# videosegmentation/video_segment

Hardware: AMD Instinct MI355X
Metric: over-segmented frames/sec at 1080p (higher is better)
Workload: dtype f32

## Files before the change

video_segment_amd/csrc/dense_graph.cpp:

```cpp
#include "dense_graph.h"
#include "scan_device.h"

#include <algorithm>
#include <chrono>
#include <cmath>
#include <cstring>
#include <atomic>
#include <functional>
#include <thread>
#include <unordered_set>

namespace vsg {

namespace {
template <class T>
DevBuf<T>& Grow(DevBuf<T>& b, size_t n) {
  if (b.size() < n) b.alloc(n + n / 2 + 1024);
  return b;
}
double NowMs() {
  using clk = std::chrono::steady_clock;
  return std::chrono::duration<double, std::milli>(clk::now().time_since_epoch()).count();
}
template <class T>
// ... 399 lines not shown
    S.seg_key = act_.seg_key;
    S.seg_cnt = act_.seg_cnt;
    S.seg_off = act_.seg_off;
    S.lead_pos = act_.lead_pos;
    S.l_ra = act_.l_ra;
    S.l_rb = act_.l_rb;
    S.l_gpos = act_.l_gpos;
    S.bk_ds = act_.bk_ds;
    S.bk_cons = act_.bk_cons;
    S.bk_flags = act_.bk_flags;
    S.cub_temp = cub_temp_.get();
    S.cub_temp_bytes = cub_temp_.size();
    S.scan = ScanScratch{scan_sums_.get(), stream_};
    S.active_cap = (int)std::min<size_t>(scratch_active_, 0x7fffffff);
  };
  bind_scratch();
  S.grow_active = [this, bind_scratch, &diag_slab_growths, &diag_slab_ms](long long need) {
    const double tg0 = NowMs();
    VSG_HIP(hipStreamSynchronize(stream_));
    VSG_HIP(hipStreamSynchronize(aux_stream_));
    VSG_HIP(hipStreamSynchronize(aux2_stream_));
    const size_t before = scratch_active_;
    EnsureActiveScratch((size_t)need);
    bind_scratch();
    ++diag_slab_growths;
    diag_slab_ms += NowMs() - tg0;
    if (getenv("VSG_DEBUG_STATS")) {
      std::fprintf(stderr, "[vsg] stage scratch: %zu -> %zu active edges (needed %lld), %.2f ms\n", before,
                   scratch_active_, need, NowMs() - tg0);
    }
    return true;
  };
  S.num_active = scalars_.get();
  S.num_segs = scalars_.get() + 1;
  S.node_key_bits = 1;
  while (S.node_key_bits < 32 && ((size_t)1 << S.node_key_bits) < N) ++S.node_key_bits;
  {
    const size_t words = 4 * ((scratch_edges_ + 255) / 256) + 4;
    S.masks.active = filter_masks_.get();
    S.masks.settled = filter_masks_.get() + words;
    S.masks.tentative = filter_masks_.get() + 2 * words;
    S.masks.block_cnt = block_cnt_.get();
    S.block_off = block_off_.get();
  }
  S.force_rollback = getenv("VSG_FORCE_ROLLBACK") ? 1 : 0;
  S.small_seg = getenv("VSG_SMALL_SEG") ? std::max(1, atoi(getenv("VSG_SMALL_SEG"))) : 24;
  S.wide_min = getenv("VSG_WIDE_MIN") ? atoi(getenv("VSG_WIDE_MIN")) : 0;
  S.wide_waves = getenv("VSG_WIDE_WAVES") ? atoi(getenv("VSG_WIDE_WAVES")) : 4;
  S.chain_relax = getenv("VSG_CHAIN_RELAX") ? atoi(getenv("VSG_CHAIN_RELAX")) : 1;
  const int hubs_default = getenv("VSG_HUBS") ? atoi(getenv("VSG_HUBS")) : 1;
  S.hubs = hubs_default;
  S.hub_excl = hub_excl_.get();
  S.hub_max_splits = getenv("VSG_HUB_SPLITS") ? std::max(0, atoi(getenv("VSG_HUB_SPLITS"))) : kHubMaxSplits;
  S.hub_cut_min_work = getenv("VSG_CUT_MIN_WORK") ? atoi(getenv("VSG_CUT_MIN_WORK")) : 0;
  S.hub_cut_ratio = getenv("VSG_CUT_RATIO") ? std::max(0, atoi(getenv("VSG_CUT_RATIO"))) : 1500;
  S.hub_check = (getenv("VSG_HUB_CHECK") && atoi(getenv("VSG_HUB_CHECK")) != 0) ? 1 : 0;
  VSG_HIP(hipMemsetAsync(hub8_.get(), 0, N, stream_));
  S.spine_min = getenv("VSG_SPINE_MIN") ? atoi(getenv("VSG_SPINE_MIN")) : 2048;
  {
    const double want = 1.15 * (double)wh_ * (double)capacity_frames_;
    const int by_graph = (int)std::min<double>(std::max<double>(want, 1 << 20), 120 << 20);
    S.spine_max_edges = getenv("VSG_SPINE_MAX_EDGES") ? atoi(getenv("VSG_SPINE_MAX_EDGES"))
                                                      : std::max(by_graph, spine_max_edges_grown_);
  }
  S.spine_off = 0;
  if (spine_limit_bucket_ != 0x7fffffff && ++spine_limit_age_ > 8) {
    spine_limit_bucket_ = 0x7fffffff;
    spine_limit_age_ = 0;
  }
  S.spine_limit_bucket = &spine_limit_bucket_;
  int spine_low_failed[2] = {0, 0}, spine_low_skip[2] = {0, 0};
  for (int b = 0; b < 2; ++b) {
    if (spine_low_cooldown_[b] > 0) {
      --spine_low_cooldown_[b];
      spine_low_skip[b] = 1;
    }
  }
  S.spine_low_failed = spine_low_failed;
  S.spine_low_skip = spine_low_skip;
  S.spine_nested_factor = getenv("VSG_SPINE_NESTED") ? std::max(1, atoi(getenv("VSG_SPINE_NESTED"))) : 1;
  S.spine_debug = getenv("VSG_SPINE_DEBUG") ? 1 : 0;
  S.spine_check = getenv("VSG_SPINE_CHECK") ? 1 : 0;
  S.rank_split_min = getenv("VSG_RANK_SPLIT_MIN") ? atoi(getenv("VSG_RANK_SPLIT_MIN")) : (1 << 20);
  S.spine_fast = getenv("VSG_SPINE_FAST") ? atoi(getenv("VSG_SPINE_FAST")) : 2;
  S.spine_fast_min = getenv("VSG_SPINE_FAST_MIN") ? atoi(getenv("VSG_SPINE_FAST_MIN")) : 32768;
  if (S.spine_min > 0) {
    const size_t ints = SpinePoolInts((size_t)S.spine_max_edges);
    if (spine_pool_.size() < ints) spine_pool_.alloc(ints);
  }
  S.spine_pool = spine_pool_.get();
  S.spine_pool_ints = spine_pool_.size();
  S.grow_spine_pool = [this, &S, &diag_spine_growths, &diag_spine_ms](long long edges) {
    if (getenv("VSG_SPINE_MAX_EDGES") || edges >= (120ll << 20)) return false;
    const long long want = std::min<long long>(edges + edges / 8, 120ll << 20);
    const long long nodes = (long long)wh_ * (long long)std::max(capacity_frames_, 1);
    const size_t ints = SpinePoolInts((size_t)want) + (size_t)(29 * std::min(want, nodes));
    if (ints <= spine_pool_.size()) return false;
    const double tg0 = NowMs();
    size_t free_b = 0, total_b = 0;
    VSG_HIP(hipMemGetInfo(&free_b, &total_b));
    if (free_b + spine_pool_.size() * sizeof(int32_t) < 2 * ints * sizeof(int32_t)) {
      int dev = 0;
      VSG_HIP(hipGetDevice(&dev));
      CacheTrim(dev);
      VSG_HIP(hipMemGetInfo(&free_b, &total_b));
      if (free_b + spine_pool_.size() * sizeof(int32_t) < 2 * ints * sizeof(int32_t)) return false;
    }
    VSG_HIP(hipStreamSynchronize(stream_));
    VSG_HIP(hipStreamSynchronize(aux_stream_));
    VSG_HIP(hipStreamSynchronize(aux2_stream_));
    spine_pool_.alloc(ints);
    ++diag_spine_growths;
    diag_spine_ms += NowMs() - tg0;
    S.spine_pool = spine_pool_.get();
    S.spine_pool_ints = spine_pool_.size();
    S.spine_max_edges = (int)want;
    spine_max_edges_grown_ = S.spine_max_edges;
    return true;
  };
  S.nmap[0] = label_uf_.get();
  S.nmap[1] = label_img_.get();
  S.nmap[2] = adjust_.get();
  S.aux_stream = aux_stream_;
  S.aux2_stream = aux2_stream_;
  S.aux_fork = aux_fork_;
  S.aux_join = aux_join_;
  S.use_rle = getenv("VSG_RLE") ? atoi(getenv("VSG_RLE")) : 1;
  S.wave_dbg = getenv("VSG_WAVE_DBG") ? atoi(getenv("VSG_WAVE_DBG")) : 0;
  S.wave_debug = (S.wave_dbg != 0 || getenv("VSG_DEBUG_STAGES") || getenv("VSG_DEBUG_STATS")) ? 1 : 0;
  optimistic_stages_ = 0;
  rollbacks_ = 0;
  S.optimistic_stages = &optimistic_stages_;
  S.rollbacks = &rollbacks_;
  S.cc = cc_.get();
  S.stats = stats_.get();
  ev_used_ = 0;
  ev_wave_.clear();
  ev_filter_.clear();
  ev_spine_.clear();
  S.ev_pool = &ev_pool_;
  S.ev_wave = &ev_wave_;
  S.ev_filter = &ev_filter_;
  S.ev_spine = &ev_spine_;
  S.ev_used = &ev_used_;
  S.mail = &mail_;
  S.zeros = &zero_pool_;
  S.main_stream = stream_;

  MergeParams P;
  P.spatial_survivors = pass == 2 ? kept_spatial_pass_.get() : nullptr;
  P.W = W_;
  P.H = H_;
  P.num_lists = L;
  P.min_region_size = min_region_size;
  P.force_merge_weight = l1_ ? 0.002f : 0.001f;
  const float scale = 2048.0f / (1.0f + 1e-6f);
  P.inv_scale = (float)(1.0 / (double)scale);
  auto largest_s = [](double t, bool inclusive) {
    auto ok = [&](float s) {
      const double r = (double)std::sqrt(s);
      return inclusive ? r <= t : r < t;
    };
    float s = (float)(t * t);
    while (!ok(s)) s = std::nextafter(s, 0.0f);
    while (ok(std::nextafter(s, 10.0f))) s = std::nextafter(s, 10.0f);
    return s;
// ... 1182 lines not shown
```

video_segment_amd/csrc/device_graph.h:

```cpp
#ifndef VSG_DEVICE_GRAPH_H_
#define VSG_DEVICE_GRAPH_H_

#include <functional>

#include "common.h"

namespace vsg {

constexpr uint8_t kFlagFinalized = 1;
constexpr uint8_t kFlagNoDesc = 2;
constexpr uint8_t kFlagTentative = 4;
constexpr uint8_t kFlagHub = 8;
constexpr uint8_t kFlagHubBroken = 16;
constexpr uint8_t kFlagHubExcluded = 32;
constexpr int kHubExclCap = 16384;
constexpr int kHubMaxAttempts = 4;
constexpr int kHubMaxSplits = 64;
constexpr int kHubCutCap = 64;
constexpr int kHubListInts = 4 + kHubExclCap + 3 * kHubCutCap;

struct NodeArrays {
  int32_t* parent;
  float4* desc_sz;
  int32_t* cons;
  uint8_t* flags;
  uint8_t* hub8;
};

struct ListDesc {
  const uint32_t* slots;
  uint8_t* kept;
  const int32_t* prev_idx;
  const int32_t* offsets;
  int32_t type;
  int32_t base_a;
  int32_t base_b;
  int32_t n;
};

struct MergeParams {
  int W, H;
  int num_lists;
  int min_region_size;
  float force_merge_weight;
  float inv_scale;
  float s_lt_005, s_lt_02, s_le_015;
  const uint8_t* spatial_survivors;
};

void UploadSpaceWeights(const float* w49, hipStream_t stream);
void LaunchMinMax(const uint8_t* bgr, size_t stride, int W, int H, int* mm, hipStream_t s);
void LaunchBilateral(const uint8_t* bgr, size_t stride, int W, int H, const float* lut,
                     float scale, float* planes, hipStream_t s);
void LaunchGaussian3(const uint8_t* bgr, size_t stride, int W, int H, float k0, float k1, float* planes,
                     hipStream_t s);
void LaunchConvertPlanar(const uint8_t* bgr, size_t stride, int W, int H, float* planes,
                         hipStream_t s);
void LaunchInterleavedToPlanar(const float* in, size_t n, float* planes, hipStream_t s);
void LaunchPlanarToInterleaved(const float* planes, size_t n, float* out, hipStream_t s);
size_t EdgeSortHistInts(size_t n_px);
size_t EdgeSortSumInts(size_t n_px);
void LaunchSpatialKeys(const float* feat, int W, int H, int l1, uint16_t* keys, int32_t* hist,
                       hipStream_t s);
void LaunchTemporalKeys(const float* cur, const float* prev, const float* flow, int W, int H,
                        int l1, int is_virtual, uint16_t* keys, int32_t* prev_idx, int32_t* hist,
                        hipStream_t s);
void LaunchBucketSort(const uint16_t* keys, size_t n_px, int per_px, int32_t* hist, int32_t* sums,
                      int32_t* offsets, uint32_t* slots_out, hipStream_t s);
void LaunchInitNodes(const float* feat, size_t n, int base, const int32_t* cons_in,
                     NodeArrays nodes, hipStream_t s);
void LaunchInitVirtualNodes(const int32_t* labels, size_t n, int base, int num_labels,
                            int32_t* first_scratch, NodeArrays nodes, hipStream_t s);

constexpr int kScanMaxTiles = 4096;
struct ScanScratch {
  int32_t* sums;
  hipStream_t owner = nullptr;
};

size_t SortPairsU32HandTempBytes(int n);
void SortPairsU32Hand(void* temp, size_t temp_bytes, const uint32_t* keys_in, uint32_t* keys_out,
                      const uint32_t* vals_in, uint32_t* vals_out, int n, int end_bit, hipStream_t s);
size_t SortPairsU32LibTempBytes(int n);
void SortPairsU32Lib(void* temp, size_t temp_bytes, const uint32_t* keys_in, uint32_t* keys_out,
                     const uint32_t* vals_in, uint32_t* vals_out, int n, int end_bit, hipStream_t s);
size_t SortPairsU32TempBytes(int n);
void SortPairsU32(void* temp, size_t temp_bytes, const uint32_t* keys_in, uint32_t* keys_out,
                  const uint32_t* vals_in, uint32_t* vals_out, int n, int end_bit, hipStream_t s);
size_t SortKeysU64TempBytes(int n);
void SortKeysU64(void* temp, size_t temp_bytes, const unsigned long long* in,
                 unsigned long long* out, int n,
                 hipStream_t s);
size_t UniqueU64TempBytes(int n);
void UniqueU64(void* temp, size_t temp_bytes, const unsigned long long* in,
               unsigned long long* out,
               int32_t* num_out, int n, hipStream_t s);

constexpr int kMailValues = 4;
struct MailSlot {
  unsigned long long* dev;
  volatile unsigned long long* host;
  unsigned seq;
// ... 13 lines not shown
  m.next = (m.next + 1) % m.slots;
  return s;
}
void MailWait(const MailSlot& slot, int count, int* values, hipStream_t s);
void MailRegisterGraph(int delta);
int MailYieldMode();
struct MailWaitCounters {
  long long waits = 0;
  double wait_ms = 0, longest_ms = 0;
};
MailWaitCounters MailWaitSnapshot();
void MailWaitResetLongest();
void LaunchMailPost(const MailSlot& slot, const int32_t* p0, const int32_t* p1, const int32_t* p2,
                    const int32_t* p3, hipStream_t s);

constexpr size_t kZeroArenaInts = 1024;
struct ZeroPool {
  int32_t* base = nullptr;
  size_t cap = 0, used = 0;
  bool second_half = false;
  size_t arena_used = 0;
};

struct FilterMasks {
  unsigned long long* active;
  unsigned long long* settled;
  unsigned long long* tentative;
  int32_t* block_cnt;
};
struct FilterSegs {
  const int32_t* start;
  const int32_t* list;
  const int32_t* pos0;
  int n;
};
struct MergeScratch {
  int active_cap;
  std::function<bool(long long need)> grow_active;
  int32_t* e_ra;
  int32_t* e_rb;
  uint32_t* e_gpos;
  int32_t* e_active;
  int32_t* e_apos;
  FilterMasks masks;
  int32_t* block_off;
  int32_t* a_ra;
  int32_t* a_rb;
  uint32_t* a_gpos;
  uint32_t* a_comp;
  uint32_t* a_idx;
  uint32_t* s_comp;
  uint32_t* s_idx;
  uint32_t* seg_key;
  int32_t* seg_cnt;
  int32_t* seg_off;
  int32_t* num_active;
  int32_t* num_segs;
  float4* bk_ds;
  int32_t* bk_cons;
  uint8_t* bk_flags;
  int force_rollback;
  int32_t* lead_pos;
  int32_t* l_ra;
  int32_t* l_rb;
  uint32_t* l_gpos;
  int use_rle;
  int group_hi;
  const int32_t* bucket_prefix;
  const int32_t* bucket_prefix_host;
  const int32_t* bucket_base_host;
  const int32_t* list_off_host;
  int32_t* seg_dev;
  size_t seg_cap;
  std::vector<int32_t>* seg_host;
  int spine_min;
  int spine_off;
  int* spine_low_failed;
  const int* spine_low_skip;
  int* spine_limit_bucket;
  int spine_nested_factor;
  int spine_max_edges;
  int spine_debug, spine_check;
  int rank_split_min;
  int spine_fast;
  int spine_fast_min;
  int32_t* spine_pool;
  size_t spine_pool_ints;
  std::function<bool(long long edges)> grow_spine_pool;
  int32_t* nmap[3];
  hipStream_t aux_stream;
  hipStream_t aux2_stream;
  hipEvent_t aux_fork, aux_join;
  int small_seg;
  int wide_min;
  int wide_waves;
  int chain_relax;
  int hubs;
  int hubs_off;
  int hub_attempt;
  int hub_splits_left;
  int hub_split_depth;
  int hub_list_dirty;
  int hub_max_splits;
  int hub_cut_min_work;
  long long hub_splits;
  const uint32_t* list_slot_base_host;
  int32_t* hub_excl;
  long long hub_retries;
  long long hub_reasons[6];
  long long hub_cuts_in_groups;
  long long hub_parts_in_later_bucket;
  long long spine_side_cuts;
  long long hub_exclusion_reruns;
  long long hub_off_reruns;
  long long group_halvings;
  long long conservative_replays;
  long long hub_cut_ratio;
  int hub_check;
  int wave_debug;
  int wave_dbg;
  int64_t* optimistic_stages;
  int64_t* rollbacks;
  int32_t* cc;
  unsigned long long* stats;
  void* cub_temp;
  size_t cub_temp_bytes;
  ScanScratch scan;
  int node_key_bits;
  std::vector<hipEvent_t>* ev_pool;
  std::vector<std::pair<int, int>>* ev_wave;
  std::vector<std::pair<int, int>>* ev_filter;
  std::vector<std::pair<int, int>>* ev_spine;
  int* ev_used;
  Mailbox* mail;
  ZeroPool* zeros;
  hipStream_t main_stream;
};
int32_t* TakeZeroed(MergeScratch& S, size_t n);

int32_t* TakeStageScalars(MergeScratch& S, size_t n);

void LaunchBuildBucketTable(const ListDesc* lists, int num_lists, int32_t* bucket_base,
                            hipStream_t s);
void LaunchInitIdentity(int32_t* a, size_t n, hipStream_t s);
struct StageInfo {
  int want_components = 0;
  int replayed = 0;
  int components = 0;
  int max_wave_segment = 0;
  int hub_stages = 0;
  long long hub_absorbed = 0;
  int hub_retries = 0;
};
void ResetHubExclusions(MergeScratch& S, NodeArrays nodes, hipStream_t s);
void RunBucketStage(int bucket, int j0, int n_b, const ListDesc* lists, const int32_t* bucket_base,
                    const uint32_t* list_slot_base, uint8_t* kept_all, NodeArrays nodes,
                    const MergeParams& P, int inert_mode, MergeScratch& S, hipStream_t s,
                    StageInfo* info = nullptr);
size_t SpinePoolInts(size_t max_edges);
void LaunchKeepVirtualBucket(const ListDesc* lists, int num_lists, hipStream_t s);

void LaunchFlatten(NodeArrays nodes, size_t n, int32_t* label_uf, hipStream_t s);
void LaunchEnforceN4(int32_t* label_img, int W, int H, const int32_t* frames_dev, int num_frames,
                     int32_t* row_flags , int32_t* adjust ,
                     hipStream_t s);
void LaunchRowRunCounts(const int32_t* label_img, int W, int H, int frame, int32_t* row_counts,
// ... 51 lines not shown
```

video_segment_amd/csrc/merge_spine.hip:

```cpp
#include <algorithm>
#include <chrono>
#include <cstdlib>
#include <cstdio>
#include <unordered_map>
#include <vector>

#include "merge_common.h"
#include "scan_device.h"

namespace vsg {

namespace {

constexpr int kNone = -1;

static inline unsigned Blocks(size_t n) { return (unsigned)((n + 255) / 256); }

__device__ __forceinline__ int CompOf(const int32_t* __restrict__ comp_base, int K, int e) {
  int lo = 0, hi = K;
  while (hi - lo > 1) {
    const int mid = (lo + hi) >> 1;
    if (comp_base[mid] <= e) lo = mid; else hi = mid;
  }
  return lo;
// ... 190 lines not shown
  int want;
  __device__ int operator()(int e) const { return state[e] == want ? 1 : 0; }
};
struct FlagScanEmit {
  int32_t* flag;
  int32_t* scan;
  __device__ void operator()(int e, int f, int before) const {
    if (flag) flag[e] = f;
    scan[e] = before;
  }
};
struct TotalPostFinish {
  int32_t* count;
  unsigned long long* mail;
  unsigned mail_seq;
  __device__ void operator()(int total) const {
    *count = total;
    MailPost(mail, mail_seq, 0, total);
  }
};

__global__ __launch_bounds__(256) void k_compact_tree(int mE, const int32_t* __restrict__ flag,
                                                       const int32_t* __restrict__ scan,
                                                       int32_t* __restrict__ te_e) {
  const int e = blockIdx.x * 256 + threadIdx.x;
  if (e < mE && flag[e]) te_e[scan[e]] = e;
}

__global__ __launch_bounds__(256) void k_arc_keys(int mt, const int32_t* __restrict__ te_e,
                                                   const int32_t* __restrict__ eu, const int32_t* __restrict__ ev,
                                                   uint32_t* __restrict__ keys, uint32_t* __restrict__ vals) {
  const int a = blockIdx.x * 256 + threadIdx.x;
  if (a >= 2 * mt) return;
  const int e = te_e[a >> 1];
  keys[a] = (uint32_t)((a & 1) ? ev[e] : eu[e]);
  vals[a] = (uint32_t)a;
}

__global__ __launch_bounds__(256) void k_arc_first(int na, const uint32_t* __restrict__ ks,
                                                    const uint32_t* __restrict__ as, int32_t* __restrict__ firstq,
                                                    int32_t* __restrict__ pos_arc) {
  const int q = blockIdx.x * 256 + threadIdx.x;
  if (q >= na) return;
  if (q == 0 || ks[q] != ks[q - 1]) firstq[ks[q]] = q;
  pos_arc[as[q]] = q;
}

__global__ __launch_bounds__(256) void k_arc_succ(int na, const uint32_t* __restrict__ ks,
                                                   const uint32_t* __restrict__ as,
                                                   const int32_t* __restrict__ firstq,
                                                   const int32_t* __restrict__ pos_arc,
                                                   const int32_t* __restrict__ te_e,
                                                   const int32_t* __restrict__ comp_base, int K,
                                                   const int32_t* __restrict__ root_vertex,
                                                   int32_t* __restrict__ succ, int32_t* __restrict__ dist) {
  const int a = blockIdx.x * 256 + threadIdx.x;
  if (a >= na) return;
  const int qb = pos_arc[a ^ 1];
  const uint32_t w = ks[qb];
  int q = qb + 1;
  if (q == na || ks[q] != w) q = firstq[w];
  int nx = (int)as[q];
  const int root = root_vertex[CompOf(comp_base, K, te_e[a >> 1])];
  if ((int)w == root && q == firstq[root]) nx = kNone;
  succ[a] = nx;
  dist[a] = nx == kNone ? 0 : 1;
}

__global__ __launch_bounds__(256) void k_rank_step(int na, const int32_t* __restrict__ s_in,
                                                    const int32_t* __restrict__ d_in, int32_t* __restrict__ s_out,
                                                    int32_t* __restrict__ d_out) {
  const int a = blockIdx.x * 256 + threadIdx.x;
  if (a >= na) return;
  const int s = s_in[a];
  if (s == kNone) {
    s_out[a] = kNone;
    d_out[a] = d_in[a];
  } else {
    s_out[a] = s_in[s];
    d_out[a] = d_in[a] + d_in[s];
  }
}

constexpr int kRankSplit = 64;
__global__ __launch_bounds__(256) void k_rank_walk(int na, int K, const int32_t* __restrict__ succ,
                                                    const int32_t* __restrict__ root_vertex,
                                                    const int32_t* __restrict__ firstq,
                                                    const uint32_t* __restrict__ as, int32_t* __restrict__ owner,
                                                    int32_t* __restrict__ local, int32_t* __restrict__ r_next,
                                                    int32_t* __restrict__ r_len) {
  const int ns0 = (na + kRankSplit - 1) / kRankSplit;
  const int t = blockIdx.x * 256 + threadIdx.x;
  if (t >= ns0 + K) return;
  int a;
  if (t < ns0) {
    a = t * kRankSplit;
  } else {
    a = (int)as[firstq[root_vertex[t - ns0]]];
    if (a % kRankSplit == 0) {
      r_next[t] = kNone;
      r_len[t] = 0;
      return;
    }
  }
  int steps = 0, cur = a, nxt;
  for (;;) {
    owner[cur] = t;
    local[cur] = steps++;
    nxt = succ[cur];
    if (nxt == kNone || nxt % kRankSplit == 0) break;
    cur = nxt;
  }
  r_next[t] = nxt == kNone ? kNone : nxt / kRankSplit;
  r_len[t] = steps;
}

__global__ __launch_bounds__(256) void k_rank_finish(int na, const int32_t* __restrict__ owner,
                                                      const int32_t* __restrict__ local,
                                                      const int32_t* __restrict__ r_dist, int32_t* __restrict__ dist) {
  const int a = blockIdx.x * 256 + threadIdx.x;
  if (a < na) dist[a] = r_dist[owner[a]] - local[a];
}

__global__ __launch_bounds__(256) void k_tree_parent(int mt, const int32_t* __restrict__ te_e,
                                                      const int32_t* __restrict__ eu,
                                                      const int32_t* __restrict__ ev,
                                                      const int32_t* __restrict__ dist, int32_t* __restrict__ child,
                                                      int32_t* __restrict__ par, int32_t* __restrict__ childidx) {
  const int j = blockIdx.x * 256 + threadIdx.x;
  if (j >= mt) return;
  const int e = te_e[j];
  const bool down = dist[2 * j] > dist[2 * j + 1];
  const int c = down ? ev[e] : eu[e];
  child[j] = c;
  par[j] = down ? eu[e] : ev[e];
  childidx[c] = j;
}

__global__ __launch_bounds__(256) void k_jump_init(int mt, const int32_t* __restrict__ te_e,
                                                    const int32_t* __restrict__ par,
                                                    const int32_t* __restrict__ childidx, int32_t* __restrict__ jump,
                                                    int32_t* __restrict__ val) {
  const int j = blockIdx.x * 256 + threadIdx.x;
  if (j >= mt) return;
  jump[j] = childidx[par[j]];
  val[j] = te_e[j];
}

__global__ __launch_bounds__(256) void k_jump_max(int mt, const int32_t* __restrict__ j_in,
                                                   const int32_t* __restrict__ v_in, int32_t* __restrict__ j_out,
                                                   int32_t* __restrict__ v_out, int32_t* __restrict__ more) {
  const int j = blockIdx.x * 256 + threadIdx.x;
  if (j >= mt) return;
  const int p = j_in[j];
  if (p == kNone) {
    j_out[j] = kNone;
    v_out[j] = v_in[j];
  } else {
    const int pp = j_in[p];
    j_out[j] = pp;
    v_out[j] = max(v_in[j], v_in[p]);
    if (more && pp != kNone) *more = 1;
  }
}

__global__ __launch_bounds__(256) void k_head_lookup(int mt, const int32_t* __restrict__ tval,
                                                      const int32_t* __restrict__ scan, int32_t* __restrict__ head) {
  const int j = blockIdx.x * 256 + threadIdx.x;
  if (j < mt) head[j] = scan[tval[j]];
}

__global__ __launch_bounds__(256) void k_classify(int mE, const int32_t* __restrict__ eu,
                                                   const int32_t* __restrict__ ev,
                                                   const int32_t* __restrict__ estate,
                                                   const int32_t* __restrict__ childidx,
                                                   const int32_t* __restrict__ head,
                                                   const int32_t* __restrict__ te_e,
                                                   int32_t* __restrict__ side_flag, int32_t* __restrict__ side_key,
                                                   int32_t* __restrict__ spine_flag) {
  const int e = blockIdx.x * 256 + threadIdx.x;
  if (e >= mE) return;
  const int ju = childidx[eu[e]], jv = childidx[ev[e]];
  const int hu = ju == kNone ? kNone : head[ju];
  const int hv = jv == kNone ? kNone : head[jv];
  const bool side = hu != kNone && hu == hv && e < te_e[hu];
  side_flag[e] = side ? 1 : 0;
  side_key[e] = side ? hu : kNone;
  bool spine = false;
  if (estate[e] == 1) {
    const int jc = (ju != kNone && te_e[ju] == e) ? ju : jv;
    spine = head[jc] == jc;
  }
  spine_flag[e] = spine ? 1 : 0;
}

__global__ __launch_bounds__(256) void k_compact_side(int mE, const int32_t* __restrict__ flag,
                                                       const int32_t* __restrict__ scan,
                                                       const int32_t* __restrict__ side_key,
                                                       uint32_t* __restrict__ keys, uint32_t* __restrict__ idx) {
  const int e = blockIdx.x * 256 + threadIdx.x;
  if (e >= mE) return;
  if (flag[e]) {
    keys[scan[e]] = (uint32_t)side_key[e];
    idx[scan[e]] = (uint32_t)e;
  }
}

__global__ __launch_bounds__(256) void k_gather_side(int n, const uint32_t* __restrict__ sorted_e,
                                                      const int32_t* __restrict__ comp_base,
                                                      const int32_t* __restrict__ comp_off, int K,
                                                      const int32_t* __restrict__ s_ra,
                                                      const int32_t* __restrict__ s_rb,
                                                      const uint32_t* __restrict__ s_gpos,
                                                      int32_t* __restrict__ o_ra, int32_t* __restrict__ o_rb,
                                                      uint32_t* __restrict__ o_gpos) {
  const int i = blockIdx.x * 256 + threadIdx.x;
  if (i >= n) return;
  const int e = (int)sorted_e[i];
  const int k = CompOf(comp_base, K, e);
  const int pos = comp_off[k] + (e - comp_base[k]);
  o_ra[i] = s_ra[pos];
  o_rb[i] = s_rb[pos];
  o_gpos[i] = s_gpos[pos];
}

struct SpineEmit {
  const int32_t* eu;
  const int32_t* ev;
  const int32_t* childidx;
  const int32_t* te_e;
  int32_t* scan;
  int32_t* sp_child;
  int32_t* sp_is_a;
  const int32_t* comp_base;
  const int32_t* comp_off;
  int K;
  __device__ void operator()(int e, int f, int before) const {
    scan[e] = before;
    if (f) {
      const int ju = childidx[eu[e]];
      const bool child_is_u = ju != kNone && te_e[ju] == e;
      sp_child[before] = child_is_u ? eu[e] : ev[e];
      const int lo = CompOf(comp_base, K, e);
      sp_is_a[before] = ((comp_off[lo] + (e - comp_base[lo])) << 1) | (child_is_u ? 1 : 0);
    }
  }
};
struct SpineFinish {
  int32_t* comp_spine;
  int K;
  __device__ void operator()(int total) const { comp_spine[K] = total; }
};
// ... 833 lines not shown
      VSG_REQUIRE(round < 32, -4, "spine: the spanning forest did not converge");
      int32_t* d_ctr = TakeZeroed(S, 16 * kAliveSlots + 4);
      int32_t* d_next_len = len_words + (len_cur ^ 1);
      hipLaunchKernelGGL(k_bor_min, dim3(Blocks(n_list)), dim3(256), 0, s, n_list, list, list_len, round, eu, ev,
                         estate, cc, best, side_key, spine_flag, d_ctr, gate, d_next_len);
      const MailSlot m_alive = NextMail(*S.mail);
      hipLaunchKernelGGL(k_bor_hook, dim3(Blocks(n_list)), dim3(256), 0, s, n_list, list, list_len, round, eu, ev,
                         estate, cc, best, side_key, spine_flag, d_ctr, m_alive.dev, m_alive.seq, gate,
                         gate_words + (round & 1));
      gate = gate_words + (round & 1);
      waiting[n_waiting++] = m_alive;
      const int depth = n_list <= ahead_max ? 1 : 0;
      const double tr0 = dbg_big ? NowMs() : 0;
      int alive = -1;
      bool complete = false;
      while (n_waiting > depth) {
        MailWait(waiting[0], 1, &alive, s);
        waiting[0] = waiting[1];
        --n_waiting;
        if (alive == 0) {
          complete = true;
          break;
        }
      }
      if (dbg_big) std::fprintf(stderr, "[vsg]   forest round %d: %d in list, %d alive, %.2f ms\n", round, n_list, alive, NowMs() - tr0);
      if (complete) break;
      const bool compact = depth == 1 ? (round >= 1 && n_list > compact_min)
                                      : (alive < n_list / 2 && n_list > compact_min);
      if (!compact) continue;
      if (!lists[0]) {
        const size_t m = pool.mark();
        const size_t cap = depth == 1 ? (size_t)n_list : (size_t)alive;
        lists[0] = pool.take(cap);
        lists[1] = pool.take(cap);
        if (!pool.ok) {
          pool.ok = true;
          pool.release(m);
          lists[0] = lists[1] = nullptr;
        }
      }
      if (!lists[0]) continue;
      hipLaunchKernelGGL(k_bor_compact, dim3(Blocks(((size_t)n_list + kBorCompactPer - 1) / kBorCompactPer)),
                         dim3(256), 0, s, n_list, list, list_len, estate, lists[which], d_next_len);
      list = lists[which];
      list_len = d_next_len;
      len_cur ^= 1;
      which ^= 1;
      if (alive >= 0) n_list = std::min(n_list, alive);
    }
    pool.release(forest_mark);
  }
  Mark(1);
  const MailSlot m_mt = NextMail(*S.mail);
  FusedScan(S.scan, StateFlagValue{estate, 1}, FlagScanEmit{flag, scan}, TotalPostFinish{scalars + 1, m_mt.dev, m_mt.seq},
            mE, s);
  int mt = 0;
  MailWait(m_mt, 1, &mt, s);
  VSG_REQUIRE(mt > 0, -4, "spine: a component without tree edges");
  const int na = 2 * mt;
  int32_t* te_e = pool.take(mt);
  int32_t* child = pool.take(mt);
  int32_t* par = pool.take(mt);
  int32_t* jump[2] = {pool.take(mt), pool.take(mt)};
  int32_t* val[2] = {pool.take(mt), pool.take(mt)};
  int32_t* head = pool.take(mt);
  int32_t* sp_child = pool.take(mt);
  int32_t* sp_is_a = pool.take(mt);
  const size_t arcs_mark = pool.mark();

  uint32_t* ak_in = reinterpret_cast<uint32_t*>(pool.take(na));
  uint32_t* av_in = reinterpret_cast<uint32_t*>(pool.take(na));
  uint32_t* ak = reinterpret_cast<uint32_t*>(pool.take(na));
  uint32_t* av = reinterpret_cast<uint32_t*>(pool.take(na));
  int32_t* pos_arc = pool.take(na);
  int32_t* succ[2] = {pool.take(na), pool.take(na)};
  int32_t* dist[2] = {pool.take(na), pool.take(na)};
  if (!pool.ok) return false;
  hipLaunchKernelGGL(k_compact_tree, dim3(Blocks(mE)), dim3(256), 0, s, mE, flag, scan, te_e);
  hipLaunchKernelGGL(k_arc_keys, dim3(Blocks(na)), dim3(256), 0, s, mt, te_e, eu, ev, ak_in, av_in);
  SortPairsU32(S.cub_temp, S.cub_temp_bytes, ak_in, ak, av_in, av, na, S.node_key_bits, s);
  hipLaunchKernelGGL(k_arc_first, dim3(Blocks(na)), dim3(256), 0, s, na, ak, av, firstq, pos_arc);
  hipLaunchKernelGGL(k_arc_succ, dim3(Blocks(na)), dim3(256), 0, s, na, ak, av, firstq, pos_arc, te_e, d_base, K,
                     root_vertex, succ[0], dist[0]);
  int cur = 0;
  bool ranked = false;
  if (na >= S.rank_split_min) {
    const int ns = (na + kRankSplit - 1) / kRankSplit + K;
    const size_t rmark = pool.mark();
    int32_t* r_next[2] = {pool.take(ns), pool.take(ns)};
    int32_t* r_len[2] = {pool.take(ns), pool.take(ns)};
    if (pool.ok) {
      int32_t* owner = succ[1];
      int32_t* local = dist[0];
      hipLaunchKernelGGL(k_rank_walk, dim3(Blocks(ns)), dim3(256), 0, s, na, K, succ[0], root_vertex, firstq, av,
                         owner, local, r_next[0], r_len[0]);
      int rc = 0;
      for (int span = 1; span < ns; span *= 2) {
        hipLaunchKernelGGL(k_rank_step, dim3(Blocks(ns)), dim3(256), 0, s, ns, r_next[rc], r_len[rc], r_next[rc ^ 1],
                           r_len[rc ^ 1]);
        rc ^= 1;
      }
      hipLaunchKernelGGL(k_rank_finish, dim3(Blocks(na)), dim3(256), 0, s, na, owner, local, r_len[rc], dist[1]);
      cur = 1;
      ranked = true;
    } else {
      pool.ok = true;
    }
    pool.release(rmark);
  }
  if (!ranked) {
    for (int span = 1; span < na; span *= 2) {
      hipLaunchKernelGGL(k_rank_step, dim3(Blocks(na)), dim3(256), 0, s, na, succ[cur], dist[cur], succ[cur ^ 1],
                         dist[cur ^ 1]);
      cur ^= 1;
    }
  }
  hipLaunchKernelGGL(k_tree_parent, dim3(Blocks(mt)), dim3(256), 0, s, mt, te_e, eu, ev, dist[cur], child, par,
                     childidx);

  Mark(2);
  hipLaunchKernelGGL(k_jump_init, dim3(Blocks(mt)), dim3(256), 0, s, mt, te_e, par, childidx, jump[0], val[0]);
  int cj = 0;
  {
    MailSlot asked = {nullptr, nullptr, 0};
    bool have_asked = false;
    for (int span = 1, step = 0; span < mt; span *= 2, ++step) {
      const bool ask = (step % 3 == 2) && span * 2 < mt;
      int32_t* d_more = ask ? TakeZeroed(S, 1) : nullptr;
      hipLaunchKernelGGL(k_jump_max, dim3(Blocks(mt)), dim3(256), 0, s, mt, jump[cj], val[cj], jump[cj ^ 1],
                         val[cj ^ 1], d_more);
      cj ^= 1;
      if (ask) {
        const MailSlot m = NextMail(*S.mail);
        LaunchMailPost(m, d_more, nullptr, nullptr, nullptr, s);
        if (have_asked) {
          int more = 0;
          MailWait(asked, 1, &more, s);
          if (!more) break;
        }
        asked = m;
        have_asked = true;
      }
    }
  }
  hipLaunchKernelGGL(k_head_lookup, dim3(Blocks(mt)), dim3(256), 0, s, mt, val[cj], scan, head);
  hipLaunchKernelGGL(k_classify, dim3(Blocks(mE)), dim3(256), 0, s, mE, eu, ev, estate, childidx, head,
                     te_e, flag, side_key, spine_flag);

  Mark(3);
  pool.release(arcs_mark);
  const MailSlot m_side = NextMail(*S.mail);
  FusedScan(S.scan, ScanLoadI32{flag}, FlagScanEmit{nullptr, scan}, TotalPostFinish{scalars + 2, m_side.dev, m_side.seq},
            mE, s);
  int n_side = 0;
  MailWait(m_side, 1, &n_side, s);
  const size_t ns = (size_t)(n_side > 0 ? n_side : 1);
  uint32_t* sk_in = reinterpret_cast<uint32_t*>(pool.take(ns));
  uint32_t* si_in = reinterpret_cast<uint32_t*>(pool.take(ns));
  uint32_t* sk = reinterpret_cast<uint32_t*>(pool.take(ns));
  uint32_t* si = reinterpret_cast<uint32_t*>(pool.take(ns));
  uint32_t* seg_key = reinterpret_cast<uint32_t*>(pool.take(ns));
  int32_t* seg_cnt = pool.take(ns);
  int32_t* seg_off = pool.take(ns);
  int32_t* o_ra = pool.take(ns);
  int32_t* o_rb = pool.take(ns);
  uint32_t* o_gpos = reinterpret_cast<uint32_t*>(pool.take(ns));
  if (!pool.ok) return false;
  hipLaunchKernelGGL(k_compact_side, dim3(Blocks(mE)), dim3(256), 0, s, mE, flag, scan, side_key, sk_in, si_in);
  FusedScan(S.scan, StateFlagValue{spine_flag, 1}, SpineEmit{eu, ev, childidx, te_e, scan, sp_child, sp_is_a, d_base, d_off, K},
            SpineFinish{comp_spine, K}, mE, s);
  hipLaunchKernelGGL(k_comp_spine, dim3(Blocks(K)), dim3(256), 0, s, K, d_base, scan, comp_spine);
  int dbg_spine_edges = 0;
  if (S.spine_debug) {
    std::vector<int32_t> cs(K + 1);
    VSG_HIP(hipMemcpy(cs.data(), comp_spine, (K + 1) * sizeof(int32_t), hipMemcpyDeviceToHost));
    dbg_spine_edges = cs[K];
  }
  Mark(4);
  if (S.spine_check) SpineSelfCheck(base, mE, eu, ev, root_vertex, side_key, spine_flag, te_e, mt);
  if (n_side > 0) {
    int side_bits = 1;
    while (side_bits < 32 && (1ll << side_bits) < (long long)mt) ++side_bits;
    SortPairsU32(S.cub_temp, S.cub_temp_bytes, sk_in, sk, si_in, si, n_side, side_bits, s);
    int32_t* d_nseg = scalars + 3;
    RunsOfSortedKeys(S.scan, sk, n_side, seg_off, seg_cnt, d_nseg, s);
    hipLaunchKernelGGL(k_gather_side, dim3(Blocks(n_side)), dim3(256), 0, s, n_side, si, d_base, d_off, K, wa.s_ra,
                       wa.s_rb, wa.s_gpos, o_ra, o_rb, o_gpos);
    WorkerArgs w2 = wa;
    w2.num_segs = d_nseg;
    w2.seg_off = seg_off;
    w2.seg_cnt = seg_cnt;
    w2.s_ra = o_ra;
    w2.s_rb = o_rb;
    w2.s_gpos = o_gpos;
    w2.T.side = 1;
    w2.s_seq = nullptr;
    VSG_REQUIRE(w2.T.hubs == 0, -4, "tree replay: a side cluster in a stage with hub regions");
    w2.work_cap = n_side / (w2.small_seg + 1) + 1;
    w2.work_list = (size_t)kWaveClasses * w2.work_cap <= ns ? seg_key : nullptr;
    w2.work_ctl = w2.work_list ? TakeZeroed(S, 2 * kWaveClasses) : nullptr;
    SpineInput nested;
    w2.wave_max = 0x7fffffff;
    if (pool.ok && depth < 8 && n_side >= S.spine_min * S.spine_nested_factor) {
      const long long room = (long long)((S.spine_pool_ints - pool_used - pool.used) / 16);
      w2.wave_max = SelectLargeSegments(n_side, d_nseg, seg_off, seg_cnt, S.spine_min * S.spine_nested_factor,
                                        room < S.spine_max_edges ? room : S.spine_max_edges, S, s, &nested,
                                        nullptr);
    }
    if (nested.segs.empty()) {
      run_workers(w2, n_side, s);
    } else {
      const int ef = NextEvent(S), ej = NextEvent(S);
      const bool fork = S.aux2_stream && ef >= 0 && ej >= 0;
      if (fork) {
        VSG_HIP(hipEventRecord((*S.ev_pool)[ef], s));
        VSG_HIP(hipStreamWaitEvent(S.aux2_stream, (*S.ev_pool)[ef], 0));
        run_workers(w2, n_side, S.aux2_stream);
        VSG_HIP(hipEventRecord((*S.ev_pool)[ej], S.aux2_stream));
      } else {
        run_workers(w2, n_side, s);
      }
      if (!RunSpineComponents(nested, w2, S, s, run_workers, pool_used + pool.used, depth + 1)) {
        WorkerArgs w3 = w2;
        w3.wave_min = w2.wave_max - 1;
        w3.wave_max = 0x7fffffff;
        w3.work_list = nullptr;
        run_workers(w3, n_side, s);
      }
      if (fork) VSG_HIP(hipStreamWaitEvent(s, (*S.ev_pool)[ej], 0));
    }
  }
  Mark(5);
  const int es0 = NextEvent(S);
  if (es0 >= 0) VSG_HIP(hipEventRecord((*S.ev_pool)[es0], s));
  int32_t* start_pos = nullptr;
  const auto LaunchSpine = [&](int max_steps) {
    hipLaunchKernelGGL(k_spine, dim3(K), dim3(64 * (1 + kSpineReaders)), 0, s, K, comp_spine, root_vertex, sp_child,
                       sp_is_a, wa.nodes, wa.T, wa.optimistic, wa.violation, wa.stats, start_pos, max_steps,
                       wa.s_gpos, wa.hub_excl);
  };
  if (S.spine_fast > 0 && mt >= S.spine_fast_min) {
    SpineFastArrays F;
    F.ck_stride = (mt >> 4) + 2 * K + 4;
    F.p = pool.take(mt);
    F.ds = reinterpret_cast<float4*>(pool.take(4 * (size_t)mt));
    F.meta = pool.take(mt);
    F.sizes = pool.take((size_t)mt + 1);
    F.pre = pool.take((size_t)mt + 1);
    F.ck = reinterpret_cast<float*>(pool.take(3 * (size_t)F.ck_stride));
    F.stop = pool.take(K);
    F.fail = pool.take(K);
    F.start_pos = pool.take(K);
    if (pool.ok) {
      start_pos = F.start_pos;
      for (int pass = 0; pass < S.spine_fast; ++pass) {
        if (pass > 0) LaunchSpine(64);
        hipLaunchKernelGGL(k_spine_fast_init, dim3((K + 63) / 64), dim3(64), 0, s, K, comp_spine, F, pass == 0 ? 1 : 0);
        hipLaunchKernelGGL(k_spine_prep, dim3(Blocks((size_t)mt + 1)), dim3(256), 0, s, mt, K, comp_spine,
                           root_vertex, sp_child, wa.nodes, wa.T, F);
        ExclusiveSum(S.scan, F.sizes, F.pre, mt + 1, s);
        hipLaunchKernelGGL(k_spine_chain, dim3(K), dim3(64 * (1 + kChProducers)), 0, s, K, comp_spine, root_vertex,
                           wa.nodes, F);
        hipLaunchKernelGGL(k_spine_verify, dim3(Blocks((size_t)F.ck_stride)), dim3(256), 0, s, K, comp_spine,
                           root_vertex, wa.nodes, wa.T, F);
        hipLaunchKernelGGL(k_spine_commit, dim3(Blocks(((size_t)mt + kCommitPer - 1) / kCommitPer)), dim3(256), 0, s, mt, K, comp_spine, root_vertex,
                           wa.nodes, F, wa.stats);
        hipLaunchKernelGGL(k_spine_finish, dim3((K + 63) / 64), dim3(64), 0, s, K, comp_spine, root_vertex,
                           wa.nodes, wa.T, F, wa.stats);
        if (S.spine_debug) {
          VSG_HIP(hipStreamSynchronize(s));
          std::vector<int32_t> cs(K + 1), sp(K), st(K), fl(K);
          VSG_HIP(hipMemcpy(cs.data(), comp_spine, (K + 1) * sizeof(int32_t), hipMemcpyDeviceToHost));
          VSG_HIP(hipMemcpy(sp.data(), F.start_pos, K * sizeof(int32_t), hipMemcpyDeviceToHost));
          VSG_HIP(hipMemcpy(st.data(), F.stop, K * sizeof(int32_t), hipMemcpyDeviceToHost));
          VSG_HIP(hipMemcpy(fl.data(), F.fail, K * sizeof(int32_t), hipMemcpyDeviceToHost));
          long long total = 0, fast = 0;
          int longest = 0, stopped = 0, failed = 0;
          for (int k = 0; k < K; ++k) {
            const int n = cs[k + 1] - cs[k];
            total += n;
            fast += sp[k];
            longest = std::max(longest, n);
            stopped += st[k] < n;
            failed += fl[k] < n;
          }
          std::fprintf(stderr, "[vsg]   streamed chain, pass %d: %lld of %lld spine steps done (longest spine %d; %d of %d "
                       "components stopped at a step that is not plain, %d at a failed test or a larger side "
                       "cluster)\n", pass, fast, total, longest, stopped, K, failed);
        }
      }
    }
  }
  LaunchSpine(0x7fffffff);
  const int es1 = NextEvent(S);
  if (es1 >= 0) {
    VSG_HIP(hipEventRecord((*S.ev_pool)[es1], s));
    if (S.ev_spine) S.ev_spine->emplace_back(es0, es1);
  }
  VSG_HIP(hipGetLastError());
  Mark(6);
  if (S.spine_debug) {
    std::fprintf(stderr, "[vsg] spine[%d]: %d components, %d edges (largest %d), %d tree edges, %d side edges, %d spine edges, "
                 "%d boruvka rounds | ms: forest %.2f rooting %.2f paths %.2f classify %.2f side %.2f spine %.2f\n",
                 depth, K, mE, in.segs[0].cnt, mt, n_side, dbg_spine_edges, dbg_rounds, tph[1] - tph[0], tph[2] - tph[1],
                 tph[3] - tph[2], tph[4] - tph[3], tph[5] - tph[4], tph[6] - tph[5]);
  }
  return true;
}

}
```

Before: 201.9.

## Rank Euler tours in LDS and find path heads with a segment tree

Adds a single-block LDS pointer-jumping kernel for list ranking when the arc count or the sampled sublist count fits in 16K entries. It also makes sampled ranking the default with an adaptive stride. It replaces the iterative pointer-jumping path-max (many launches plus host mailbox waits) with a segment tree over Euler-tour positions: each tree edge does atomicMax range updates and each query walks up to the root. This cuts kernel launches and host syncs, at the cost of atomic contention and of reusing the ak_in buffer as tree storage, which assumes it is large enough.

```diff
diff --git a/video_segment_amd/csrc/dense_graph.cpp b/video_segment_amd/csrc/dense_graph.cpp
--- a/video_segment_amd/csrc/dense_graph.cpp
+++ b/video_segment_amd/csrc/dense_graph.cpp
@@ -505,6 +505,9 @@
   S.spine_debug = getenv("VSG_SPINE_DEBUG") ? 1 : 0;
   S.spine_check = getenv("VSG_SPINE_CHECK") ? 1 : 0;
   S.rank_split_min = getenv("VSG_RANK_SPLIT_MIN") ? atoi(getenv("VSG_RANK_SPLIT_MIN")) : (1 << 20);
+  S.root_fast = getenv("VSG_ROOT_FAST") ? atoi(getenv("VSG_ROOT_FAST")) : 1;
+  S.rank_lds_max = getenv("VSG_RANK_LDS_MAX") ? std::min(std::max(atoi(getenv("VSG_RANK_LDS_MAX")), 0), kRankLdsMax)
+                                              : kRankLdsMax;
   S.spine_fast = getenv("VSG_SPINE_FAST") ? atoi(getenv("VSG_SPINE_FAST")) : 2;
   S.spine_fast_min = getenv("VSG_SPINE_FAST_MIN") ? atoi(getenv("VSG_SPINE_FAST_MIN")) : 32768;
   if (S.spine_min > 0) {
diff --git a/video_segment_amd/csrc/device_graph.h b/video_segment_amd/csrc/device_graph.h
--- a/video_segment_amd/csrc/device_graph.h
+++ b/video_segment_amd/csrc/device_graph.h
@@ -18,6 +18,7 @@
 constexpr int kHubMaxSplits = 64;
 constexpr int kHubCutCap = 64;
 constexpr int kHubListInts = 4 + kHubExclCap + 3 * kHubCutCap;
+constexpr int kRankLdsMax = 16384;
 
 struct NodeArrays {
   int32_t* parent;
@@ -197,6 +198,8 @@
   int spine_max_edges;
   int spine_debug, spine_check;
   int rank_split_min;
+  int root_fast;
+  int rank_lds_max;
   int spine_fast;
   int spine_fast_min;
   int32_t* spine_pool;
diff --git a/video_segment_amd/csrc/merge_spine.hip b/video_segment_amd/csrc/merge_spine.hip
--- a/video_segment_amd/csrc/merge_spine.hip
+++ b/video_segment_amd/csrc/merge_spine.hip
@@ -296,22 +296,23 @@
   }
 }
 
-constexpr int kRankSplit = 64;
-__global__ __launch_bounds__(256) void k_rank_walk(int na, int K, const int32_t* __restrict__ succ,
+constexpr int kRankSplitLog2 = 6;
+__global__ __launch_bounds__(256) void k_rank_walk(int na, int K, int split_log2, const int32_t* __restrict__ succ,
                                                     const int32_t* __restrict__ root_vertex,
                                                     const int32_t* __restrict__ firstq,
                                                     const uint32_t* __restrict__ as, int32_t* __restrict__ owner,
                                                     int32_t* __restrict__ local, int32_t* __restrict__ r_next,
                                                     int32_t* __restrict__ r_len) {
-  const int ns0 = (na + kRankSplit - 1) / kRankSplit;
+  const int split_mask = (1 << split_log2) - 1;
+  const int ns0 = (na + split_mask) >> split_log2;
   const int t = blockIdx.x * 256 + threadIdx.x;
   if (t >= ns0 + K) return;
   int a;
   if (t < ns0) {
-    a = t * kRankSplit;
+    a = t << split_log2;
   } else {
     a = (int)as[firstq[root_vertex[t - ns0]]];
-    if (a % kRankSplit == 0) {
+    if ((a & split_mask) == 0) {
       r_next[t] = kNone;
       r_len[t] = 0;
       return;
@@ -322,10 +323,10 @@
     owner[cur] = t;
     local[cur] = steps++;
     nxt = succ[cur];
-    if (nxt == kNone || nxt % kRankSplit == 0) break;
+    if (nxt == kNone || (nxt & split_mask) == 0) break;
     cur = nxt;
   }
-  r_next[t] = nxt == kNone ? kNone : nxt / kRankSplit;
+  r_next[t] = nxt == kNone ? kNone : nxt >> split_log2;
   r_len[t] = steps;
 }
 
@@ -334,6 +335,52 @@
                                                       const int32_t* __restrict__ r_dist, int32_t* __restrict__ dist) {
   const int a = blockIdx.x * 256 + threadIdx.x;
   if (a < na) dist[a] = r_dist[owner[a]] - local[a];
+}
+
+constexpr int kRankLdsThreads = 1024;
+constexpr int kRankLdsPer = kRankLdsMax / kRankLdsThreads;
+static_assert(kRankLdsPer * kRankLdsThreads == kRankLdsMax, "kRankLdsMax: a multiple of the block");
+__global__ __launch_bounds__(kRankLdsThreads) void k_rank_lds(int n, const int32_t* __restrict__ s_in,
+                                                               const int32_t* __restrict__ d_in,
+                                                               int32_t* __restrict__ d_out) {
+  __shared__ int32_t nx[kRankLdsMax];
+  __shared__ int32_t ds[kRankLdsMax];
+  for (int i = threadIdx.x; i < n; i += kRankLdsThreads) {
+    nx[i] = s_in[i];
+    ds[i] = d_in[i];
+  }
+  __syncthreads();
+  for (;;) {
+    int sv[kRankLdsPer], dv[kRankLdsPer];
+    int active = 0;
+#pragma unroll
+    for (int k = 0; k < kRankLdsPer; ++k) {
+      const int i = threadIdx.x + k * kRankLdsThreads;
+      sv[k] = kNone;
+      dv[k] = 0;
+      if (i < n) {
+        const int sn = nx[i];
+        dv[k] = ds[i];
+        if (sn != kNone) {
+          sv[k] = nx[sn];
+          dv[k] += ds[sn];
+          active = 1;
+        }
+      }
+    }
+    const int more = __syncthreads_or(active);
+    if (!more) break;
+#pragma unroll
+    for (int k = 0; k < kRankLdsPer; ++k) {
+      const int i = threadIdx.x + k * kRankLdsThreads;
+      if (i < n) {
+        nx[i] = sv[k];
+        ds[i] = dv[k];
+      }
+    }
+    __syncthreads();
+  }
+  for (int i = threadIdx.x; i < n; i += kRankLdsThreads) d_out[i] = ds[i];
 }
 
 __global__ __launch_bounds__(256) void k_tree_parent(int mt, const int32_t* __restrict__ te_e,
@@ -382,6 +429,47 @@
                                                       const int32_t* __restrict__ scan, int32_t* __restrict__ head) {
   const int j = blockIdx.x * 256 + threadIdx.x;
   if (j < mt) head[j] = scan[tval[j]];
+}
+
+__global__ __launch_bounds__(256) void k_tree_parent_tx(int mt, const int32_t* __restrict__ te_e,
+                                                         const int32_t* __restrict__ eu,
+                                                         const int32_t* __restrict__ ev,
+                                                         const int32_t* __restrict__ dist,
+                                                         const int32_t* __restrict__ comp_base, int K,
+                                                         const int32_t* __restrict__ scan, int N,
+                                                         int32_t* __restrict__ tree, int32_t* __restrict__ qpos,
+                                                         int32_t* __restrict__ child, int32_t* __restrict__ par,
+                                                         int32_t* __restrict__ childidx) {
+  const int j = blockIdx.x * 256 + threadIdx.x;
+  if (j >= mt) return;
+  const int e = te_e[j];
+  const int d0 = dist[2 * j], d1 = dist[2 * j + 1];
+  const bool down = d0 > d1;
+  const int c = down ? ev[e] : eu[e];
+  child[j] = c;
+  par[j] = down ? eu[e] : ev[e];
+  childidx[c] = j;
+  const int base = 2 * scan[comp_base[CompOf(comp_base, K, e)]];
+  const int hi = base + (down ? d0 : d1);
+  const int lo = base + (down ? d1 : d0) + 1;
+  qpos[j] = hi;
+  int l = lo + N, r = hi + N + 1;
+  while (l < r) {
+    if (l & 1) atomicMax(&tree[l++], e);
+    if (r & 1) atomicMax(&tree[--r], e);
+    l >>= 1;
+    r >>= 1;
+  }
+}
+
+__global__ __launch_bounds__(256) void k_path_head(int mt, const int32_t* __restrict__ qpos, int N,
+                                                    const int32_t* __restrict__ tree,
+                                                    const int32_t* __restrict__ scan, int32_t* __restrict__ head) {
+  const int j = blockIdx.x * 256 + threadIdx.x;
+  if (j >= mt) return;
+  int m = -1;
+  for (int x = qpos[j] + N; x >= 1; x >>= 1) m = max(m, tree[x]);
+  head[j] = scan[m];
 }
 
 __global__ __launch_bounds__(256) void k_classify(int mE, const int32_t* __restrict__ eu,
@@ -1381,27 +1469,48 @@
   hipLaunchKernelGGL(k_arc_first, dim3(Blocks(na)), dim3(256), 0, s, na, ak, av, firstq, pos_arc);
   hipLaunchKernelGGL(k_arc_succ, dim3(Blocks(na)), dim3(256), 0, s, na, ak, av, firstq, pos_arc, te_e, d_base, K,
                      root_vertex, succ[0], dist[0]);
+  const bool fast = S.root_fast != 0;
+  const int lds_max = S.rank_lds_max;
   int cur = 0;
   bool ranked = false;
-  if (na >= S.rank_split_min) {
-    const int ns = (na + kRankSplit - 1) / kRankSplit + K;
+  int dbg_rank = 0, dbg_split = 0;
+  if (fast && na <= lds_max && na < S.rank_split_min) {
+    hipLaunchKernelGGL(k_rank_lds, dim3(1), dim3(kRankLdsThreads), 0, s, na, succ[0], dist[0], dist[1]);
+    cur = 1;
+    ranked = true;
+    dbg_rank = 1;
+  } else if (na >= S.rank_split_min || fast) {
+    int split_log2 = kRankSplitLog2;
+    if (fast) {
+      split_log2 = 1;
+      while (split_log2 < kRankSplitLog2 && ((na + (1 << split_log2) - 1) >> split_log2) + K > lds_max) ++split_log2;
+    }
+    const int ns = ((na + (1 << split_log2) - 1) >> split_log2) + K;
+    const bool lds = fast && ns <= lds_max;
     const size_t rmark = pool.mark();
     int32_t* r_next[2] = {pool.take(ns), pool.take(ns)};
     int32_t* r_len[2] = {pool.take(ns), pool.take(ns)};
     if (pool.ok) {
       int32_t* owner = succ[1];
       int32_t* local = dist[0];
-      hipLaunchKernelGGL(k_rank_walk, dim3(Blocks(ns)), dim3(256), 0, s, na, K, succ[0], root_vertex, firstq, av,
-                         owner, local, r_next[0], r_len[0]);
+      hipLaunchKernelGGL(k_rank_walk, dim3(Blocks(ns)), dim3(256), 0, s, na, K, split_log2, succ[0], root_vertex,
+                         firstq, av, owner, local, r_next[0], r_len[0]);
       int rc = 0;
-      for (int span = 1; span < ns; span *= 2) {
-        hipLaunchKernelGGL(k_rank_step, dim3(Blocks(ns)), dim3(256), 0, s, ns, r_next[rc], r_len[rc], r_next[rc ^ 1],
-                           r_len[rc ^ 1]);
-        rc ^= 1;
+      if (lds) {
+        hipLaunchKernelGGL(k_rank_lds, dim3(1), dim3(kRankLdsThreads), 0, s, ns, r_next[0], r_len[0], r_len[1]);
+        rc = 1;
+      } else {
+        for (int span = 1; span < ns; span *= 2) {
+          hipLaunchKernelGGL(k_rank_step, dim3(Blocks(ns)), dim3(256), 0, s, ns, r_next[rc], r_len[rc],
+                             r_next[rc ^ 1], r_len[rc ^ 1]);
+          rc ^= 1;
+        }
       }
       hipLaunchKernelGGL(k_rank_finish, dim3(Blocks(na)), dim3(256), 0, s, na, owner, local, r_len[rc], dist[1]);
       cur = 1;
       ranked = true;
+      dbg_rank = lds ? 3 : 2;
+      dbg_split = 1 << split_log2;
     } else {
       pool.ok = true;
     }
@@ -1414,35 +1523,51 @@
       cur ^= 1;
     }
   }
-  hipLaunchKernelGGL(k_tree_parent, dim3(Blocks(mt)), dim3(256), 0, s, mt, te_e, eu, ev, dist[cur], child, par,
-                     childidx);
+  int32_t* tree = nullptr;
+  int tree_n = 1;
+  if (fast) {
+    while (tree_n < na + 1) tree_n *= 2;
+    tree = reinterpret_cast<int32_t*>(ak_in);
+    VSG_HIP(hipMemsetAsync(tree, 0xff, 2 * (size_t)tree_n * sizeof(int32_t), s));
+    hipLaunchKernelGGL(k_tree_parent_tx, dim3(Blocks(mt)), dim3(256), 0, s, mt, te_e, eu, ev, dist[cur], d_base, K,
+                       scan, tree_n, tree, jump[0], child, par, childidx);
+  } else {
+    hipLaunchKernelGGL(k_tree_parent, dim3(Blocks(mt)), dim3(256), 0, s, mt, te_e, eu, ev, dist[cur], child, par,
+                       childidx);
+  }
 
   Mark(2);
-  hipLaunchKernelGGL(k_jump_init, dim3(Blocks(mt)), dim3(256), 0, s, mt, te_e, par, childidx, jump[0], val[0]);
-  int cj = 0;
-  {
-    MailSlot asked = {nullptr, nullptr, 0};
-    bool have_asked = false;
-    for (int span = 1, step = 0; span < mt; span *= 2, ++step) {
-      const bool ask = (step % 3 == 2) && span * 2 < mt;
-      int32_t* d_more = ask ? TakeZeroed(S, 1) : nullptr;
-      hipLaunchKernelGGL(k_jump_max, dim3(Blocks(mt)), dim3(256), 0, s, mt, jump[cj], val[cj], jump[cj ^ 1],
-                         val[cj ^ 1], d_more);
-      cj ^= 1;
-      if (ask) {
-        const MailSlot m = NextMail(*S.mail);
-        LaunchMailPost(m, d_more, nullptr, nullptr, nullptr, s);
-        if (have_asked) {
-          int more = 0;
-          MailWait(asked, 1, &more, s);
-          if (!more) break;
-        }
-        asked = m;
-        have_asked = true;
-      }
-    }
-  }
-  hipLaunchKernelGGL(k_head_lookup, dim3(Blocks(mt)), dim3(256), 0, s, mt, val[cj], scan, head);
+  int dbg_jumps = 0;
+  if (fast) {
+    hipLaunchKernelGGL(k_path_head, dim3(Blocks(mt)), dim3(256), 0, s, mt, jump[0], tree_n, tree, scan, head);
+  } else {
+    hipLaunchKernelGGL(k_jump_init, dim3(Blocks(mt)), dim3(256), 0, s, mt, te_e, par, childidx, jump[0], val[0]);
+    int cj = 0;
+    {
+      MailSlot asked = {nullptr, nullptr, 0};
+      bool have_asked = false;
+      for (int span = 1, step = 0; span < mt; span *= 2, ++step) {
+        const bool ask = (step % 3 == 2) && span * 2 < mt;
+        int32_t* d_more = ask ? TakeZeroed(S, 1) : nullptr;
+        hipLaunchKernelGGL(k_jump_max, dim3(Blocks(mt)), dim3(256), 0, s, mt, jump[cj], val[cj], jump[cj ^ 1],
+                           val[cj ^ 1], d_more);
+        cj ^= 1;
+        ++dbg_jumps;
+        if (ask) {
+          const MailSlot m = NextMail(*S.mail);
+          LaunchMailPost(m, d_more, nullptr, nullptr, nullptr, s);
+          if (have_asked) {
+            int more = 0;
+            MailWait(asked, 1, &more, s);
+            if (!more) break;
+          }
+          asked = m;
+          have_asked = true;
+        }
+      }
+    }
+    hipLaunchKernelGGL(k_head_lookup, dim3(Blocks(mt)), dim3(256), 0, s, mt, val[cj], scan, head);
+  }
   hipLaunchKernelGGL(k_classify, dim3(Blocks(mE)), dim3(256), 0, s, mE, eu, ev, estate, childidx, head,
                      te_e, flag, side_key, spine_flag);
 
@@ -1600,9 +1725,13 @@
   Mark(6);
   if (S.spine_debug) {
     std::fprintf(stderr, "[vsg] spine[%d]: %d components, %d edges (largest %d), %d tree edges, %d side edges, %d spine edges, "
-                 "%d boruvka rounds | ms: forest %.2f rooting %.2f paths %.2f classify %.2f side %.2f spine %.2f\n",
+                 "%d boruvka rounds | ms: forest %.2f rooting %.2f paths %.2f classify %.2f side %.2f spine %.2f | "
+                 "rank %s (stride %d), %s\n",
                  depth, K, mE, in.segs[0].cnt, mt, n_side, dbg_spine_edges, dbg_rounds, tph[1] - tph[0], tph[2] - tph[1],
-                 tph[3] - tph[2], tph[4] - tph[3], tph[5] - tph[4], tph[6] - tph[5]);
+                 tph[3] - tph[2], tph[4] - tph[3], tph[5] - tph[4], tph[6] - tph[5],
+                 dbg_rank == 1 ? "lds" : dbg_rank == 2 ? "sampled+global" : dbg_rank == 3 ? "sampled+lds" : "global",
+                 dbg_split, fast ? "paths by intervals" : "paths by jumps");
+    if (!fast) std::fprintf(stderr, "[vsg]   paths: %d jump steps\n", dbg_jumps);
   }
   return true;
 }
```

Measured after the change: 200.3 (median of 2 runs). No clear change (-0.8%).
